# SiTronXD/vk3dGaussianSplatting

Hardware: AMD Instinct MI355X
Metric: Msplats/s + total frame ms (InitSortList/RadixSort/FindRanges/Render split) (higher is better)
Workload: dtype f32; 1 GPU; Garden-30k shape: 5,834,784 gaussians @ 1920x1080; num_gaussians=5834784, width=1920, height=1080, render_mode=exact, render_kernel=auto, sort_algorithm=radix4, frames_in_flight=1, parallelism=single GPU

## Files before the change

### vk3dgaussiansplatting_amd/csrc/gs_debug.cpp

```cpp
#include "gs_ctx.h"

using namespace gs;

extern "C" {

int gs_debug_init_sort_list(gs_ctx* c, const float view[16], const float proj[16],
                            const float cam_pos[3], uint32_t sh_mode) {
    if (!c) return GS_ERR_INVALID;
    const bool outputs_valid = c->outputs_valid;
    list_launching(c);
    if (!c->n || !c->capacity) return fail(c, GS_ERR_NO_SCENE, "gs_debug_init_sort_list: scene/resolution not set");
    if (!view || !proj || !cam_pos || sh_mode > 2u) return fail(c, GS_ERR_INVALID, "gs_debug_init_sort_list: bad argument");
    HIP_TRY(c, hipSetDevice(c->device));
    FrameParams fp = make_frame_params(c, view, proj, cam_pos, sh_mode);
    fp.parity = (c->emit_parity ^= 1u);
    launch_project(fp, c->scene, c->scratch, c->stream);
    launch_scan_blocks(fp, c->scratch, c->sort.params, c->ranges, c->sort.coarse, c->stream);
    launch_emit(fp, c->scratch, c->sort, c->stream);
    if (int r = check_launch(c, "InitSortList")) return r;
    HIP_TRY(c, hipStreamSynchronize(c->stream));
    unsorted_list_ready(c, fp, outputs_valid);
    SortParams sp{};
    HIP_TRY(c, hipMemcpy(&sp, c->sort.params, sizeof(sp), hipMemcpyDeviceToHost));
    return sp.overflow ? GS_WARN_OVERFLOW : GS_OK;
}

static int read_tile_words(gs_ctx* c, const uint32_t* dev, uint32_t num_elems, void* dst, size_t bytes) {
    if (bytes > (size_t)num_elems * sizeof(uint32_t)) return fail(c, GS_ERR_INVALID, "gs_debug_read: size exceeds buffer");
    const size_t cnt = bytes / sizeof(uint32_t);
    uint32_t* out = static_cast<uint32_t*>(dst);
    if (c->hi16) {
        std::vector<uint16_t> h(num_elems);
        if (num_elems) HIP_TRY(c, hipMemcpy(h.data(), dev, (size_t)num_elems * sizeof(uint16_t), hipMemcpyDeviceToHost));
        for (size_t i = 0; i < cnt; ++i) out[i] = h[i];
    } else if (cnt) {
        HIP_TRY(c, hipMemcpy(out, dev, cnt * sizeof(uint32_t), hipMemcpyDeviceToHost));
    }
    for (size_t i = 0; i < cnt; ++i) {
        const uint32_t k = out[i] / c->grid_w, x = out[i] - k * c->grid_w;
        out[i] = (c->first_row + k * c->row_stride) * c->grid_w + x;
    }
    return GS_OK;
}

int gs_debug_read(gs_ctx* c, int which, void* dst, size_t bytes) {
    if (!c || !dst) return GS_ERR_INVALID;
    HIP_TRY(c, hipSetDevice(c->device));
    HIP_TRY(c, hipStreamSynchronize(c->stream));
    if (c->last.kind == LastFrame::kNone && which != GS_BUF_IMAGE) return fail(c, GS_ERR_NO_SCENE, "gs_debug_read: no frame rendered yet");
    SortParams sp{};
    HIP_TRY(c, hipMemcpy(&sp, c->sort.params, sizeof(sp), hipMemcpyDeviceToHost));
    const size_t e_bytes = (size_t)sp.num_elems * sizeof(uint32_t);
    const void* src = nullptr;
    size_t avail = 0;
    const int si = c->last.sorted_index;
    switch (which) {
        case GS_BUF_SORTED_TILE:
            return read_tile_words(c, c->sort.hi[si], sp.num_elems, dst, bytes);
        case GS_BUF_SORTED_DEPTH:
            if (c->last.kind == LastFrame::kFrame && c->cfg.sort_algorithm != GS_SORT_TILE_BUCKET) {
                if (bytes > e_bytes) return fail(c, GS_ERR_INVALID, "gs_debug_read: size exceeds buffer");
                std::vector<uint32_t> ids(sp.num_elems), depth(c->n);
                if (sp.num_elems) HIP_TRY(c, hipMemcpy(ids.data(), c->sort.id[si], e_bytes, hipMemcpyDeviceToHost));
                HIP_TRY(c, hipMemcpy(depth.data(), c->scratch.depth_key, (size_t)c->n * sizeof(uint32_t), hipMemcpyDeviceToHost));
                uint32_t* out = static_cast<uint32_t*>(dst);
                for (size_t i = 0; i < bytes / sizeof(uint32_t); ++i) out[i] = ids[i] < c->n ? depth[ids[i]] : 0u;
                return GS_OK;
            }
            src = c->sort.lo[si]; avail = e_bytes; break;
        case GS_BUF_SORTED_ID: src = c->sort.id[si]; avail = e_bytes; break;
        case GS_BUF_RANGES: src = c->ranges; avail = (size_t)c->grid_w * c->grid_h * 8; break;
        case GS_BUF_COUNT: {
            if (bytes > sizeof(uint64_t)) return fail(c, GS_ERR_INVALID, "gs_debug_read: size");
            std::memcpy(dst, &sp.counter, bytes);
            return GS_OK;
        }
        case GS_BUF_IMAGE: src = c->framebuffer; avail = (size_t)c->width * c->height * 4; break;
        case GS_BUF_UNSORTED_TILE:
        case GS_BUF_UNSORTED_DEPTH:
        case GS_BUF_UNSORTED_ID:
            if (c->last.kind != LastFrame::kUnsortedList)
                return fail(c, GS_ERR_INVALID, "gs_debug_read: unsorted list only valid after gs_debug_init_sort_list");
            if (which == GS_BUF_UNSORTED_TILE) return read_tile_words(c, c->sort.hi[0], sp.num_elems, dst, bytes);
            src = which == GS_BUF_UNSORTED_DEPTH ? c->sort.lo[0] : c->sort.id[0];
            avail = e_bytes;
            break;
        case GS_BUF_COLOR:
        case GS_BUF_COV: {
            const size_t need = (size_t)c->n * 4 * sizeof(float);
            if (bytes > need) return fail(c, GS_ERR_INVALID, "gs_debug_read: size exceeds buffer");
            std::vector<SplatRaster> host(c->n);
            HIP_TRY(c, hipMemcpy(host.data(), c->scratch.raster, (size_t)c->n * sizeof(SplatRaster), hipMemcpyDeviceToHost));
            std::vector<float> opacity;
            std::vector<uint32_t> touched;
            std::vector<float> on_demand;
            const bool whole_grid = c->row_begin == 0u && c->row_end == c->grid_h && c->row_stride == 1u;
            if (which == GS_BUF_COLOR) {
                opacity.resize(c->n); touched.resize(c->n);
                HIP_TRY(c, hipMemcpy(opacity.data(), c->scene.opacity, (size_t)c->n * sizeof(float), hipMemcpyDeviceToHost));
                HIP_TRY(c, hipMemcpy(touched.data(), c->scratch.tiles_touched, (size_t)c->n * sizeof(uint32_t), hipMemcpyDeviceToHost));
                if (whole_grid) {
                    float* dev = nullptr;
                    HIP_TRY(c, hipMalloc((void**)&dev, need));
                    launch_debug_colour(c->last.fp, c->scene, c->scratch, dev, c->stream);
                    hipError_t e = hipGetLastError();
                    if (e == hipSuccess) e = hipStreamSynchronize(c->stream);
                    on_demand.resize((size_t)c->n * 4);
                    if (e == hipSuccess) e = hipMemcpy(on_demand.data(), dev, need, hipMemcpyDeviceToHost);
                    (void)hipFree(dev);
                    HIP_TRY(c, e);
                }
            }
            std::vector<uint8_t> wrote((size_t)c->num_blocks * 4);
            HIP_TRY(c, hipMemcpy(wrote.data(), c->scratch.wave_wrote, wrote.size(), hipMemcpyDeviceToHost));
            std::vector<float> outv((size_t)c->n * 4, 0.0f);
            for (uint32_t i = 0; i < c->n; ++i) {
                if (!wrote[i / 64u]) continue;
                const SplatRaster& r = host[i];
                float* o = &outv[(size_t)i * 4];
                if (which == GS_BUF_COLOR) {
                    if (touched[i]) { o[0] = r.r; o[1] = r.g; o[2] = r.b; o[3] = opacity[i]; }
                    else if (!on_demand.empty() && on_demand[(size_t)i * 4 + 3] != 0.0f) {
                        o[0] = on_demand[(size_t)i * 4]; o[1] = on_demand[(size_t)i * 4 + 1]; o[2] = on_demand[(size_t)i * 4 + 2]; o[3] = opacity[i];
                    }
                }
                else { o[0] = r.cx; o[1] = r.cy; o[2] = r.cz; o[3] = 0.0f; }
            }
            std::memcpy(dst, outv.data(), bytes);
            return GS_OK;
        }
        default: return fail(c, GS_ERR_INVALID, "gs_debug_read: unknown buffer id");
    }
    if (bytes > avail) return fail(c, GS_ERR_INVALID, "gs_debug_read: size exceeds buffer");
    if (bytes) HIP_TRY(c, hipMemcpy(dst, src, bytes, hipMemcpyDeviceToHost));
    return GS_OK;
}

int gs_sort_host(gs_ctx* c, uint32_t* tile, uint32_t* depth, uint32_t* id, uint32_t n,
                 uint32_t num_sort_bits) {
    if (!c || !tile || !depth || !id) return GS_ERR_INVALID;
    if (num_sort_bits == 0 || num_sort_bits > 64 || (num_sort_bits % kRadixBits) != 0)
        return fail(c, GS_ERR_INVALID, "gs_sort_host: num_sort_bits must be a multiple of 4 in [4,64]");
    if (n == 0) return GS_OK;
    HIP_TRY(c, hipSetDevice(c->device));
    SortBuffers sb{};
    DeviceOwner mem;
    int rc = alloc_sort(c, mem, sb, n);
    if (rc != GS_OK) { mem.release(); return rc; }
    const size_t bytes = (size_t)n * sizeof(uint32_t);
    hipError_t e = hipMemcpyAsync(sb.hi[0], tile, bytes, hipMemcpyHostToDevice, c->stream);
    if (e == hipSuccess) e = hipMemcpyAsync(sb.lo[0], depth, bytes, hipMemcpyHostToDevice, c->stream);
    if (e == hipSuccess) e = hipMemcpyAsync(sb.id[0], id, bytes, hipMemcpyHostToDevice, c->stream);
    int si = 0;
    if (e == hipSuccess) {
        launch_set_sort_params(sb.params, sb.coarse, n, c->stream);
        si = launch_radix_sort(sb, whole_list_run(c, n, num_sort_bits), c->stream);
        e = si < 0 ? hipErrorInvalidValue : hipGetLastError();
    }
    if (e == hipSuccess) e = hipMemcpyAsync(tile, sb.hi[si], bytes, hipMemcpyDeviceToHost, c->stream);
    if (e == hipSuccess) e = hipMemcpyAsync(depth, sb.lo[si], bytes, hipMemcpyDeviceToHost, c->stream);
    if (e == hipSuccess) e = hipMemcpyAsync(id, sb.id[si], bytes, hipMemcpyDeviceToHost, c->stream);
    if (e == hipSuccess) e = hipStreamSynchronize(c->stream);
    mem.release();
    if (e != hipSuccess) return fail(c, GS_ERR_HIP, std::string("gs_sort_host: ") + hipGetErrorString(e));
    return GS_OK;
}

int gs_sort_bench(gs_ctx* c, uint32_t n, uint32_t num_tiles, uint32_t iters, uint64_t seed,
                  float* ms_per_sort, uint32_t* sorted_ok) {
    if (!c || !ms_per_sort || n == 0 || num_tiles == 0 || iters == 0) return GS_ERR_INVALID;
    HIP_TRY(c, hipSetDevice(c->device));
    SortBuffers sb{};
    DeviceOwner mem;
    int rc = alloc_sort(c, mem, sb, n);
    if (rc != GS_OK) { mem.release(); return rc; }
    const SortRun run = whole_list_run(c, n, num_sort_bits_for(num_tiles));
    uint32_t* bad = nullptr;
    hipEvent_t e0 = nullptr, e1 = nullptr;
    hipError_t e = mem.alloc(bad, sizeof(uint32_t));
    if (e == hipSuccess) e = hipEventCreate(&e0);
    if (e == hipSuccess) e = hipEventCreate(&e1);
    float total_ms = 0.0f;
    int si = 0;
    for (uint32_t it = 0; it < iters + 1 && e == hipSuccess; ++it) {
        launch_fill_random_keys(sb.lo[0], sb.hi[0], sb.id[0], n, num_tiles, seed + it, c->stream);
        launch_set_sort_params(sb.params, sb.coarse, n, c->stream);
        e = hipEventRecord(e0, c->stream);
        if (e != hipSuccess) break;
        si = launch_radix_sort(sb, run, c->stream);
        if (si < 0) { si = 0; e = hipErrorInvalidValue; break; }
        e = hipEventRecord(e1, c->stream);
        if (e == hipSuccess) e = hipStreamSynchronize(c->stream);
        float ms = 0.0f;
        if (e == hipSuccess) e = hipEventElapsedTime(&ms, e0, e1);
        if (it > 0) total_ms += ms;
    }
    uint32_t bad_host = 0;
    if (e == hipSuccess) e = hipMemsetAsync(bad, 0, sizeof(uint32_t), c->stream);
    if (e == hipSuccess) {
        launch_check_sorted(sb.lo[si], sb.hi[si], n, bad, c->stream);
        e = hipMemcpyAsync(&bad_host, bad, sizeof(uint32_t), hipMemcpyDeviceToHost, c->stream);
    }
    if (e == hipSuccess) e = hipStreamSynchronize(c->stream);
    if (e0) (void)hipEventDestroy(e0);
    if (e1) (void)hipEventDestroy(e1);
    mem.release();
    if (e != hipSuccess) return fail(c, GS_ERR_HIP, std::string("gs_sort_bench: ") + hipGetErrorString(e));
    *ms_per_sort = total_ms / (float)iters;
    if (sorted_ok) *sorted_ok = bad_host == 0 ? 1u : 0u;
// ... 39 lines not shown
```

### vk3dgaussiansplatting_amd/csrc/gs_internal.h

```cpp
#pragma once

#include <hip/hip_runtime.h>
#include <stdint.h>
#include "gs_record.h"

namespace gs {

constexpr int kWave = 64;
constexpr int kTile = 16;
constexpr int kRadixBits = 4;
constexpr int kBins = 1 << kRadixBits;

constexpr int kSortThreads = 256;
constexpr int kSortKeysPerThread = 8;
constexpr int kSortTile = kSortThreads * kSortKeysPerThread;
constexpr int kSegments = 512;
constexpr int kCoarse = 64;
constexpr int kMaxSortPasses = 16;
#ifndef GS_FED_MAX_GROUPS
#define GS_FED_MAX_GROUPS 1024
#endif
constexpr uint32_t kFedMaxGroups = GS_FED_MAX_GROUPS;

constexpr int kBins8 = 256;
// ... 67 lines not shown
    uint32_t* block_sums;
    uint32_t* block_offsets;
    uint2* help_list;
    uint32_t* help_count;
    uint32_t* help_slot;
    uint32_t* band_list;
    uint32_t* block_flags;
    uint32_t* flag_offsets;
    uint32_t* sorted_sums;
    SortParams* aux_params;
    uint32_t* elems_note;
    float* view_z;
};
#ifndef GS_EMIT_SLICE
#define GS_EMIT_SLICE 4096
#endif
constexpr uint32_t kEmitSlice = GS_EMIT_SLICE;
constexpr uint32_t kEmitHelpCap = 65536;
constexpr uint32_t kEmitNoHelp = 0xFFFFFFFFu;
__host__ __device__ inline uint32_t emit_helpers(uint32_t capacity) {
    const uint32_t by_capacity = capacity / kEmitSlice + 1u;
    return by_capacity < kEmitHelpCap ? by_capacity : kEmitHelpCap;
}

struct SortBuffers {
    uint32_t *lo[2], *hi[2], *id[2];
    uint32_t* table;
    uint32_t* seg_sum;
    uint32_t* coarse;
    uint32_t* fed[3];
    SortParams* params;
    uint32_t digit_bits;
};

struct SortRun {
    uint32_t capacity = 0;
    uint32_t first_bit = 0;
    uint32_t num_sort_bits = 0;
    int start = 0;
    uint32_t coarse_pass = 0;
    const SortParams* params = nullptr;
    bool drop_depth_payload = false;
    bool hi16 = false;
    float share = 1.0f;
    bool fed = false;
    hipEvent_t* scatter_events = nullptr;
};

struct SortPass {
    uint32_t shift;
    uint32_t bits, mask;
    bool tile_word;
    bool word16;
    uint32_t word_shift;
    int lo_in, lo_out;
    bool last;
};
inline uint32_t sort_pass_count(const SortRun& r, uint32_t digit_bits) {
    return r.num_sort_bits > r.first_bit ? (r.num_sort_bits - r.first_bit + digit_bits - 1u) / digit_bits : 0u;
}
inline SortPass sort_pass(const SortRun& r, uint32_t digit_bits, uint32_t k) {
    SortPass p{};
    p.shift = r.first_bit + k * digit_bits;
    p.bits = r.num_sort_bits - p.shift < digit_bits ? r.num_sort_bits - p.shift : digit_bits;
    p.mask = (1u << p.bits) - 1u;
    p.tile_word = p.shift >= 32u;
    p.last = p.shift + digit_bits >= r.num_sort_bits;
    p.lo_in = 4; p.lo_out = 4;
    if (r.drop_depth_payload) {
        if (p.tile_word) { p.lo_in = 0; p.lo_out = 0; }
        else if (r.first_bit == 0u) {
            p.lo_in = p.shift >= 16u ? 2 : 4;
            p.lo_out = p.shift + digit_bits >= 32u ? 0 : (p.shift + digit_bits >= 16u ? 2 : 4);
        }
    }
    const bool lo16 = !p.tile_word && p.lo_in == 2;
    p.word16 = (p.tile_word && r.hi16) || lo16;
    p.word_shift = lo16 ? p.shift - 16u : p.shift & 31u;
    return p;
}

void launch_project(const FrameParams& fp, const SceneBuffers& scene, const SplatScratch& sc,
                    hipStream_t stream);
void launch_debug_colour(const FrameParams& fp, const SceneBuffers& scene, const SplatScratch& sc, float* out_rgba, hipStream_t stream);
void launch_scan_blocks(const FrameParams& fp, const SplatScratch& sc, SortParams* params,
                        uint32_t* ranges, uint32_t* coarse, hipStream_t stream);
void launch_emit(const FrameParams& fp, const SplatScratch& sc, const SortBuffers& sb,
                 hipStream_t stream);
void launch_splat_list(const FrameParams& fp, const SplatScratch& sc, const SortBuffers& sb, hipStream_t stream);
void launch_gather_sorted(const FrameParams& fp, const SplatScratch& sc, const SortBuffers& sb, int sorted, hipStream_t stream);
void launch_emit_sorted(const FrameParams& fp, const SplatScratch& sc, const SortBuffers& sb, int sorted, hipStream_t stream);
int launch_radix_sort(const SortBuffers& sb, const SortRun& run, hipStream_t stream);
int launch_radix_sort8(const SortBuffers& sb, const SortRun& run, hipStream_t stream);
int init_tile_sort();
void launch_tile_sort(const FrameParams& fp, const uint32_t* ranges, uint32_t* lo, uint32_t* id,
                      uint32_t* lo_alt, uint32_t* id_alt, hipStream_t stream, hipStream_t helper = nullptr,
                      hipEvent_t fork = nullptr, hipEvent_t join = nullptr);
void launch_find_ranges(const FrameParams& fp, const uint32_t* sorted_tile, const SortParams* params,
                        uint32_t* ranges, hipStream_t stream);
void launch_tile_order(const FrameParams& fp, const uint32_t* ranges, uint32_t* order, hipStream_t stream);
size_t tile_order_words(uint32_t grid_w, uint32_t grid_h);
struct RenderOutputs {
    float4* rgba32f;
    float* depth;
    const float* view_z;
};
void launch_render(const FrameParams& fp, const SplatRaster* raster, const uint32_t* sorted_id,
                   const uint32_t* ranges, const uint32_t* order, uint8_t* rgba, uint32_t render_mode,
                   uint32_t render_kernel, hipStream_t stream, const RenderOutputs& outs = RenderOutputs{});
struct SplatScan {
    uint32_t* offsets;
    uint32_t* block_sums;
    uint32_t* block_offsets;
    uint32_t* totals;
};
constexpr int kRowFloats = 10;
struct BackwardBuffers {
    float* rows;
    SplatScan scan;
    uint32_t* vis_ids;
};
inline const uint32_t* visible_count_of(const BackwardBuffers& bb) { return bb.scan.totals + 1; }
inline size_t backward_row_bytes(uint32_t capacity) { return (size_t)capacity * kRowFloats * sizeof(float); }
inline uint32_t backward_blocks(uint32_t n) { return (n + 255u) / 256u; }
struct BackwardFrame {
    FrameParams fp;
    SceneBuffers scene;
    SplatScratch sc;
    const uint32_t* sorted_id;
    const uint32_t* ranges;
    BackwardBuffers bb;
};
void launch_backward(const BackwardFrame& f, const float* grad_rgba, const float* grad_depth, float* grad_records,
                     hipStream_t stream);
void launch_backward_visible_scan(const BackwardFrame& f, uint32_t* ids_out, uint32_t max_rows, uint32_t* count_out,
                                  hipStream_t stream);
void launch_backward_visible_rows(const BackwardFrame& f, const float* grad_rgba, const float* grad_depth,
                                  uint32_t max_rows, float* grad_rows, hipStream_t stream);
size_t backward_camera_partial_bytes(uint32_t n);
void launch_backward_camera(const BackwardFrame& f, float* partials, float* grad_camera, hipStream_t stream);
struct LossBuffers {
    float* maps;
    float* tile_sums;
};
size_t loss_map_bytes(uint32_t width, uint32_t height);
size_t loss_tile_bytes(uint32_t width, uint32_t height);
void launch_photometric_loss(const LossBuffers& lb, const float* rgba, const float* target, float lambda, const float* bg,
                             uint32_t width, uint32_t height, float* loss_out, float* grad, hipStream_t stream);
void launch_aos_to_soa(const float* chunk, uint32_t first, uint32_t count, uint32_t n,
                       const SceneBuffers& s, hipStream_t stream);
void launch_block_bounds(uint32_t n, const SceneBuffers& s, hipStream_t stream);
void launch_upload_rows(const float* records, uint32_t n, const uint32_t* ids, const uint32_t* count, uint32_t max_rows,
                        const SceneBuffers& s, hipStream_t stream);
struct AdamStep {
    float beta1, beta2, c1, c2, eps;
    float step[6], lo[6], hi[6];
};
void launch_adam_rows(float* records, float* m, float* v, uint32_t n, const uint32_t* ids, const float* grad_rows,
                      const uint32_t* count, uint32_t max_rows, const AdamStep& a, hipStream_t stream);
void launch_adam_rows_raw(float* raw, float* records, float* m, float* v, uint32_t n, const uint32_t* ids,
                          const float* grad_rows, const uint32_t* count, uint32_t max_rows, const AdamStep& a,
                          hipStream_t stream);
void launch_convert_space(const float* src, float* dst, uint32_t n, bool to_raw, hipStream_t stream);
void launch_reset_opacity_raw(float* raw, float* records, float* m, float* v, uint32_t n, float max_opacity, float logit,
                              hipStream_t stream);
struct DensifyStatsArgs {
    const uint32_t* ids;
// ... 55 lines not shown
```

### vk3dgaussiansplatting_amd/csrc/gs_project.hip

```cpp
#include <cstdlib>
#include "gs_splat_math.h"

namespace gs {

__device__ __forceinline__ Mat3 mat3_mul(const Mat3& a, const Mat3& b) {
    Mat3 c;
#pragma unroll
    for (int j = 0; j < 3; ++j)
#pragma unroll
        for (int i = 0; i < 3; ++i) {
            float acc = a.m[0][i] * b.m[j][0];
            acc = acc + a.m[1][i] * b.m[j][1];
            acc = acc + a.m[2][i] * b.m[j][2];
            c.m[j][i] = acc;
        }
    return c;
}
__device__ __forceinline__ Mat3 mat3_transpose(const Mat3& a) {
    Mat3 t;
#pragma unroll
    for (int j = 0; j < 3; ++j)
#pragma unroll
        for (int i = 0; i < 3; ++i) t.m[j][i] = a.m[i][j];
    return t;
// ... 176 lines not shown
    const bool survives = leader && mask != 0xFu;
    if (leader && !survives) {
        sc.block_sums[b] = 0u;
        if (fp.splat_first) sc.block_flags[b] = 0u;
        reinterpret_cast<uint32_t*>(sc.wave_wrote)[b] = 0u;
    }
    const uint64_t vote = __ballot(survives);
    if (lane == 0) s_cnt[wave] = (uint32_t)__builtin_popcountll(vote);
    __syncthreads();
    uint32_t before = 0u, total = 0u;
#pragma unroll
    for (int w = 0; w < kCullThreads / 64; ++w) {
        const uint32_t c = s_cnt[w];
        before += w < wave ? c : 0u;
        total += c;
    }
    if (total == 0u) return;
    if (threadIdx.x == 0) s_base = atomicAdd(&sc.help_count[2u + fp.parity], total);
    __syncthreads();
    if (survives)
        sc.band_list[s_base + before + (uint32_t)__builtin_popcountll(vote & ((1ull << lane) - 1ull))] = b | (mask << 28);
}

template <bool NT>
__device__ __forceinline__ float sh_load(const float* p) { return NT ? __builtin_nontemporal_load(p) : *p; }

template <bool NT>
__device__ __forceinline__ void splat_colour(const FrameParams& fp, const float* shp, const uint32_t n, const float px, const float py,
                                             const float pz, float res[3]) {
    const float ddx = px - fp.cam_pos[0], ddy = py - fp.cam_pos[1], ddz = pz - fp.cam_pos[2];
    const float len = sqrtf(ddx * ddx + ddy * ddy + ddz * ddz);
    float basis[16];
    sh_eval4(ddx / len, ddy / len, ddz / len, basis);
    res[0] = 0.0f; res[1] = 0.0f; res[2] = 0.0f;
    if (fp.sh_mode == 0u) {
#pragma unroll
        for (int i = 0; i < 16; ++i)
#pragma unroll
            for (int c = 0; c < 3; ++c)
                res[c] = res[c] + sh_load<NT>(shp + (size_t)(i * 3 + c) * n) * basis[i];
    } else if (fp.sh_mode == 1u) {
#pragma unroll
        for (int i = 1; i < 16; ++i)
#pragma unroll
            for (int c = 0; c < 3; ++c)
                res[c] = res[c] + sh_load<NT>(shp + (size_t)(i * 3 + c) * n) * basis[i];
#pragma unroll
        for (int c = 0; c < 3; ++c) res[c] = res[c] - 0.5f;
    } else if (fp.sh_mode == 2u) {
#pragma unroll
        for (int c = 0; c < 3; ++c) res[c] = res[c] + sh_load<NT>(shp + (size_t)c * n) * basis[0];
    }
#pragma unroll
    for (int c = 0; c < 3; ++c) {
        res[c] = res[c] + 0.5f;
        res[c] = maxf(res[c], 0.0f);
    }
}

#ifndef GS_PROJECT_MINBLOCKS
#define GS_PROJECT_MINBLOCKS 7
#endif
template <bool NT_SH, bool VIEW_Z>
__global__ __launch_bounds__(kProjThreads, GS_PROJECT_MINBLOCKS) void k_project(const FrameParams fp,
                                                           const SceneBuffers scene,
                                                           const SplatScratch sc, const uint32_t num_blocks) {
    __shared__ uint32_t s_wave_sum[kProjThreads / 64];
    __shared__ uint32_t s_wave_emits[kProjThreads / 64];
    __shared__ uint32_t s_wave_flags[kProjThreads / 64];
    __shared__ float4 s_raster[kProjThreads * 3];
    const uint32_t n = fp.num_gaussians;
    const bool band = !owns_every_row(fp);
    const bool listed = band && fp.row_stride == 1u;
    uint32_t blk = blockIdx.x;
    bool wave_skip = false;
    if (listed) {
        if (blk >= sc.help_count[2u + fp.parity]) return;
        const uint32_t rec = sc.band_list[blk];
        blk = rec & 0x0FFFFFFFu;
        wave_skip = ((rec >> 28) >> wave_id()) & 1u;
    }
    const uint32_t g = blk * kProjThreads + threadIdx.x;
    uint32_t count = 0;
    bool kept = false;
    float4 rec0 = make_float4(0.f, 0.f, 0.f, 0.f), rec1 = rec0, rec2 = rec0;

    if (g < n && !wave_skip) {
        const float px = scene.pos[g], py = scene.pos[(size_t)n + g], pz = scene.pos[2 * (size_t)n + g];
        float vp[4];
        mat4_mul_vec4(fp.view, px, py, pz, 1.0f, vp);
        if (!(-vp[2] <= fp.near_plane)) {
            float q[4];
            mat4_mul_vec4(fp.proj, vp[0], vp[1], vp[2], vp[3], q);
            const float ndc_x = q[0] / q[3];
            const float ndc_y = q[1] / q[3];
            if (!(fabsf(ndc_x) > fp.ndc_cull || fabsf(ndc_y) > fp.ndc_cull)) {
                float nd = (-vp[2] - fp.near_plane) / (fp.far_plane - fp.near_plane);
                nd = clampf(nd, 0.0f, 1.0f);
                const uint32_t depth_key = f2u_sat(nd * 4294967296.0f);
                bool band_skip = false;

                if (band) {
                    const float hgt = (float)fp.height;
                    const float tfx = fp.tan_fov_y * (float)fp.width / hgt;
                    const float tx = clampf(vp[0] / vp[2], -tfx * fp.in_view_limit, tfx * fp.in_view_limit);
                    const float ty = clampf(vp[1] / vp[2], -fp.tan_fov_y * fp.in_view_limit, fp.tan_fov_y * fp.in_view_limit);
                    const float rmax = radius_bound(fp, tx, ty, vp[2], scene.sig2[g]);
                    const float sy_b = (1.0f - ndc_y) * 0.5f * hgt;
                    band_skip = misses_owned_rows(fp, sy_b - rmax, sy_b + rmax);
                }
                if (!band_skip) {
                    float scale[3], rot[4], cov[3];
#pragma unroll
                    for (int a = 0; a < 3; ++a) scale[a] = scene.scale[a * (size_t)n + g];
#pragma unroll
                    for (int a = 0; a < 4; ++a) rot[a] = scene.rot[a * (size_t)n + g];
                    get_covariance(fp, scale, rot, vp, cov);

                    float sx = ndc_x, sy = -ndc_y;
                    sx = (sx + 1.0f) * 0.5f;
                    sy = (sy + 1.0f) * 0.5f;
                    sx = sx * (float)fp.width;
                    sy = sy * (float)fp.height;

                    const float det = cov[0] * cov[2] - cov[1] * cov[1];
                    const float radius = tile_extent_radius(cov[0], cov[1], cov[2]);
                    const int gw = (int)fp.grid_w, gh = (int)fp.grid_h;
                    const int min_x = clampi(f2i_sat((sx - radius) / 16.0f), 0, gw);
                    const int min_y = clampi(f2i_sat((sy - radius) / 16.0f), 0, gh);
                    int tx = f2i_sat((sx + radius) / 16.0f);
                    int ty = f2i_sat((sy + radius) / 16.0f);
                    const int max_x = clampi(tx == 2147483647 ? tx : tx + 1, 0, gw);
                    const int max_y = clampi(ty == 2147483647 ? ty : ty + 1, 0, gh);

                    int y0 = min_y > (int)fp.row_begin ? min_y : (int)fp.row_begin;
                    int y1 = max_y < (int)fp.row_end ? max_y : (int)fp.row_end;
                    if (y1 < y0) y1 = y0;
                    const int k0 = owned_rows_below(fp, y0), k1 = owned_rows_below(fp, y1);
                    count = (uint32_t)(max_x - min_x) * (uint32_t)(k1 - k0);

                    kept = true;
                    rec0 = make_float4(sx, sy, 0.0f, 0.0f);
                    rec2 = make_float4(0.0f, cov[0], cov[1], cov[2]);
                    if (count != 0u) {
                        float opacity = scene.opacity[g];
                        float inv_x = 0.0f, inv_y = 0.0f, inv_z = 0.0f;
                        if (det != 0.0f) {
                            const float det_inv = 1.0f / det;
                            inv_x = cov[2] * det_inv;
                            inv_y = -cov[1] * det_inv;
                            inv_z = cov[0] * det_inv;
                        } else {
                            opacity = 0.0f;
                        }
                        rec0.z = inv_x; rec0.w = inv_y;
                        rec2.x = opacity;
                        float res[3];
                        splat_colour<NT_SH>(fp, scene.sh + g, n, px, py, pz, res);
                        rec1 = make_float4(inv_z, res[0], res[1], res[2]);
                        sc.depth_key[g] = depth_key;
                        if constexpr (VIEW_Z) sc.view_z[g] = -vp[2];
                        sc.extents[g] = make_uint2((uint32_t)min_x | ((uint32_t)k0 << 16),
                                                   (uint32_t)max_x | ((uint32_t)k1 << 16));
                    }
                }
            }
        }
        sc.tiles_touched[g] = count;
    } else if (g < n) {
        sc.tiles_touched[g] = 0u;
    }

    s_raster[threadIdx.x * 3 + 0] = rec0;
    s_raster[threadIdx.x * 3 + 1] = rec1;
    s_raster[threadIdx.x * 3 + 2] = rec2;
    const uint32_t wsum = wave_sum_to_lane63(count);
    const uint32_t wflags = (uint32_t)__popcll(__ballot(count != 0u));
    const bool wave_kept = __ballot(kept) != 0ull;
    if (lane_id() == 63) {
        s_wave_sum[wave_id()] = wsum;
        s_wave_flags[wave_id()] = wflags;
#ifndef GS_PROJECT_WRITE_ALL
#define GS_PROJECT_WRITE_ALL 0
#endif
        const uint32_t wrote = (band ? wsum != 0u : (GS_PROJECT_WRITE_ALL || wave_kept)) ? 1u : 0u;
        s_wave_emits[wave_id()] = wrote;
        sc.wave_wrote[blk * (kProjThreads / 64) + wave_id()] = (uint8_t)wrote;
    }
    __syncthreads();
    {
        const uint32_t first = blk * kProjThreads;
        const uint32_t valid = (n - first) < (uint32_t)kProjThreads ? (n - first) : (uint32_t)kProjThreads;
        float4* out = reinterpret_cast<float4*>(sc.raster + first);
#pragma unroll
        for (int q = 0; q < 3; ++q) {
            const uint32_t i = q * kProjThreads + threadIdx.x;
            if (i < valid * 3u && s_wave_emits[i / 192u]) out[i] = s_raster[i];
        }
    }
    uint32_t t = 0;
#pragma unroll
    for (int w = 0; w < kProjThreads / 64; ++w) t += s_wave_sum[w];
    if (threadIdx.x == 0) {
        sc.block_sums[blk] = t;
        if (fp.splat_first) sc.block_flags[blk] = s_wave_flags[0] + s_wave_flags[1] + s_wave_flags[2] + s_wave_flags[3];
    }
    if (!fp.splat_first) register_emit_helpers(fp, sc, blk, t);
}

struct ScanJob { const uint32_t* sums; uint32_t* offsets; SortParams* params; uint32_t capacity;
                 uint32_t* host_note; };
constexpr uint32_t kScanClearWgs = 8;
__global__ __launch_bounds__(1024) void k_scan_blocks(const ScanJob job0, const ScanJob job1, uint32_t jobs, uint32_t num_blocks,
                                                       uint4* __restrict__ zero_a, uint32_t n16_a,
                                                       uint4* __restrict__ zero_b, uint32_t n16_b,
                                                       uint32_t* __restrict__ next_help_count) {
    if (blockIdx.x >= jobs) {
        const uint32_t k = blockIdx.x - jobs;
        if (k == 0u && threadIdx.x == 0 && next_help_count) { next_help_count[0] = 0u; next_help_count[2] = 0u; }
        for (uint32_t i = k * 1024u + threadIdx.x; i < n16_a; i += kScanClearWgs * 1024u) zero_a[i] = make_uint4(0u, 0u, 0u, 0u);
        for (uint32_t i = k * 1024u + threadIdx.x; i < n16_b; i += kScanClearWgs * 1024u) zero_b[i] = make_uint4(0u, 0u, 0u, 0u);
        return;
    }
    const ScanJob job = blockIdx.x == 0 ? job0 : job1;
    const uint32_t* __restrict__ block_sums = job.sums;
    uint32_t* __restrict__ block_offsets = job.offsets;
    SortParams* params = job.params;
    const uint32_t capacity = job.capacity;
    __shared__ uint64_t s_wave_tot[16];
    const int tid = threadIdx.x, lane = tid & 63, wave = tid >> 6;
    const uint32_t per = (((num_blocks + 1023u) / 1024u) + 3u) & ~3u;
    const uint4* in4 = reinterpret_cast<const uint4*>(block_sums + (size_t)tid * per);
    uint4* out4 = reinterpret_cast<uint4*>(block_offsets + (size_t)tid * per);
    auto sat = [](uint64_t x) { return (uint32_t)(x > 0xFFFFFFFFull ? 0xFFFFFFFFull : x); };
    constexpr uint32_t kHeld = 8;
    const bool held = per / 4 <= kHeld;
    uint4 v[kHeld];
    uint64_t sum = 0;
    if (held) {
#pragma unroll
        for (uint32_t i = 0; i < kHeld; ++i) v[i] = i < per / 4 ? in4[i] : make_uint4(0u, 0u, 0u, 0u);
#pragma unroll
        for (uint32_t i = 0; i < kHeld; ++i) sum += (uint64_t)v[i].x + v[i].y + v[i].z + v[i].w;
    } else {
#pragma unroll 4
        for (uint32_t i = 0; i < per / 4; ++i) {
            const uint4 w = in4[i];
            sum += (uint64_t)w.x + w.y + w.z + w.w;
        }
    }
    const uint64_t inc = wave_inclusive_scan64(sum);
    if (lane == 63) s_wave_tot[wave] = inc;
    __syncthreads();
    uint64_t run = inc - sum;
    for (int w = 0; w < wave; ++w) run += s_wave_tot[w];
    if (tid == 1023) {
        const uint64_t counter = run + sum;
        const uint32_t e = counter < capacity ? (uint32_t)counter : capacity;
        params->counter = counter;
        params->num_elems = e;
        params->num_groups = (e + kSortTile - 1) / kSortTile;
        params->groups_per_seg = (params->num_groups + kSegments - 1) / kSegments;
        params->overflow = counter > capacity ? 1u : 0u;
        if (job.host_note) __hip_atomic_store(job.host_note, e + 1u, __ATOMIC_RELAXED, __HIP_MEMORY_SCOPE_SYSTEM);
    }
    if (held) {
#pragma unroll
        for (uint32_t i = 0; i < kHeld; ++i) {
// ... 80 lines not shown
    __syncthreads();

    const uint32_t g0 = blk * kProjThreads;
    const uint32_t my_excl = s_incl[tid] - cnt;
    const uint32_t c_begin = slice * kEmitSlice;
    const uint32_t c_end = alone || total - c_begin < kEmitSlice ? total : c_begin + kEmitSlice;
    for (uint32_t c0 = c_begin; c0 < c_end; c0 += kEmitChunk) {
#pragma unroll
        for (int k = 0; k < kEmitChunk / kProjThreads; ++k) s_owner[k * kProjThreads + tid] = 0u;
        __syncthreads();
        if (cnt != 0u) {
            if (my_excl >= c0) {
                if (my_excl - c0 < (uint32_t)kEmitChunk) s_owner[my_excl - c0] = (uint32_t)tid + 1u;
            } else if (my_excl + cnt > c0) {
                s_owner[0] = (uint32_t)tid + 1u;
            }
        }
        __syncthreads();
        uint4 o = *reinterpret_cast<const uint4*>(&s_owner[4 * tid]);
        o.y = o.y > o.x ? o.y : o.x;
        o.z = o.z > o.y ? o.z : o.y;
        o.w = o.w > o.z ? o.w : o.z;
        const uint32_t winc = wave_inclusive_max(o.w);
        if (lane_id() == 63) s_wmax[wave_id()] = winc;
        uint32_t prev = __shfl_up(winc, 1, 64);
        if (lane_id() == 0) prev = 0u;
        __syncthreads();
        for (int w = 0; w < wave_id(); ++w) prev = prev > s_wmax[w] ? prev : s_wmax[w];
        o.x = o.x > prev ? o.x : prev;
        o.y = o.y > prev ? o.y : prev;
        o.z = o.z > prev ? o.z : prev;
        o.w = o.w > prev ? o.w : prev;
        *reinterpret_cast<uint4*>(&s_owner[4 * tid]) = o;
        __syncthreads();
#pragma unroll
        for (int k = 0; k < kEmitChunk / kProjThreads; ++k) {
            const uint32_t jj = (uint32_t)(k * kProjThreads + tid);
            const uint32_t j = c0 + jj;
            if (j < total) {
                const uint32_t s = s_owner[jj] - 1u;
                const uint32_t excl = s > 0u ? s_incl[s - 1u] : 0u;
                const uint32_t id_local = j - excl;
                const uint2 ext = s_ext[s];
                const uint32_t min_x = ext.x & 0xFFFFu, y0 = ext.x >> 16, max_x = ext.y & 0xFFFFu;
                const uint32_t wdt = max_x - min_x;
                uint32_t ry = (uint32_t)((float)id_local * __builtin_amdgcn_rcpf((float)wdt));
                int32_t rx = (int32_t)(id_local - ry * wdt);
                if (rx < 0) { --ry; rx += (int32_t)wdt; }
                else if ((uint32_t)rx >= wdt) { ++ry; rx -= (int32_t)wdt; }
                const uint32_t tile_key = (y0 + ry) * fp.grid_w + (min_x + (uint32_t)rx);
                const uint64_t out = (uint64_t)base + j;
                if (out < fp.capacity) {
                    if (fp.hi16) reinterpret_cast<uint16_t*>(out_hi)[out] = (uint16_t)tile_key;
                    else out_hi[out] = tile_key;
                    if constexpr (SORTED) out_id[out] = s_depth[s];
                    else { out_lo[out] = s_depth[s]; out_id[out] = g0 + s; }
                }
            }
        }
        __syncthreads();
    }
}

void launch_project(const FrameParams& fp, const SceneBuffers& scene, const SplatScratch& sc,
                    hipStream_t stream) {
    const uint32_t blocks = (fp.num_gaussians + kProjThreads - 1) / kProjThreads;
    if (blocks == 0) return;
    const bool listed = !(fp.row_begin == 0u && fp.row_end == fp.grid_h) && fp.row_stride == 1u;
    if (listed) hipLaunchKernelGGL(k_band_cull, dim3((blocks * 4u + (uint32_t)kCullThreads - 1u) / (uint32_t)kCullThreads), dim3(kCullThreads), 0, stream,
                                   fp, scene, sc, blocks);
#ifndef GS_PROJECT_NT_SH_ABOVE
#define GS_PROJECT_NT_SH_ABOVE ((size_t)256u << 20)
#endif
    const bool nt_sh = (size_t)fp.num_gaussians * 236u > GS_PROJECT_NT_SH_ABOVE;
    if (sc.view_z) {
        if (nt_sh) hipLaunchKernelGGL((k_project<true, true>), dim3(blocks), dim3(kProjThreads), 0, stream, fp, scene, sc, blocks);
        else hipLaunchKernelGGL((k_project<false, true>), dim3(blocks), dim3(kProjThreads), 0, stream, fp, scene, sc, blocks);
    } else {
        if (nt_sh) hipLaunchKernelGGL((k_project<true, false>), dim3(blocks), dim3(kProjThreads), 0, stream, fp, scene, sc, blocks);
        else hipLaunchKernelGGL((k_project<false, false>), dim3(blocks), dim3(kProjThreads), 0, stream, fp, scene, sc, blocks);
    }
}

__global__ __launch_bounds__(256) void k_debug_colour(const FrameParams fp, const SceneBuffers scene, const SplatScratch sc, float4* out) {
    const uint32_t n = fp.num_gaussians;
    const uint32_t g = blockIdx.x * 256u + threadIdx.x;
    if (g >= n) return;
    float4 o = make_float4(0.f, 0.f, 0.f, 0.f);
    if (sc.wave_wrote[g >> 6] && sc.raster[g].cx != 0.0f && sc.tiles_touched[g] == 0u) {
        float res[3];
        splat_colour<false>(fp, scene.sh + g, n, scene.pos[g], scene.pos[(size_t)n + g], scene.pos[2 * (size_t)n + g], res);
        o = make_float4(res[0], res[1], res[2], 1.0f);
    }
    out[g] = o;
}

void launch_debug_colour(const FrameParams& fp, const SceneBuffers& scene, const SplatScratch& sc, float* out_rgba, hipStream_t stream) {
    const uint32_t blocks = (fp.num_gaussians + 255u) / 256u;
    if (blocks) hipLaunchKernelGGL(k_debug_colour, dim3(blocks), dim3(256), 0, stream, fp, scene, sc, reinterpret_cast<float4*>(out_rgba));
}

void launch_scan_blocks(const FrameParams& fp, const SplatScratch& sc, SortParams* params,
                        uint32_t* ranges, uint32_t* coarse, hipStream_t stream) {
    const uint32_t blocks = (fp.num_gaussians + kProjThreads - 1) / kProjThreads;
    const uint32_t n16_ranges = (fp.grid_w * fp.grid_h * 2u + 3u) / 4u;
    const uint32_t n16_coarse = (uint32_t)(kMaxSortPasses * kBins * kCoarse) / 4u;
    const ScanJob elements{sc.block_sums, sc.block_offsets, params, fp.capacity, sc.elems_note};
    const ScanJob splats{sc.block_flags, sc.flag_offsets, sc.aux_params, fp.num_gaussians, nullptr};
    const uint32_t jobs = fp.splat_first ? 2u : 1u;
    hipLaunchKernelGGL(k_scan_blocks, dim3(jobs + kScanClearWgs), dim3(1024), 0, stream, elements, splats, jobs, blocks,
                       reinterpret_cast<uint4*>(ranges), n16_ranges, reinterpret_cast<uint4*>(coarse), n16_coarse,
                       sc.help_count + (fp.parity ^ 1u));
}

void launch_emit(const FrameParams& fp, const SplatScratch& sc, const SortBuffers& sb,
                 hipStream_t stream) {
    const uint32_t blocks = (fp.num_gaussians + kProjThreads - 1) / kProjThreads;
    if (blocks == 0) return;
    const uint32_t helpers = emit_helpers(fp.capacity);
    hipLaunchKernelGGL((k_emit<false>), dim3(helpers + blocks), dim3(kProjThreads), 0, stream, fp, sc, sb.lo[0],
                       sb.hi[0], sb.id[0], blocks, helpers, (const uint32_t*)nullptr, (const uint32_t*)nullptr);
}

__global__ __launch_bounds__(kProjThreads) void k_splat_list(const FrameParams fp, const SplatScratch sc,
                                                              uint32_t* __restrict__ out_depth, uint32_t* __restrict__ out_count,
                                                              uint32_t* __restrict__ out_id) {
    __shared__ uint32_t s_cnt[kProjThreads / 64], s_flag[kProjThreads / 64];
    const uint32_t blk = blockIdx.x, g = blk * kProjThreads + threadIdx.x;
    if (blk == 0u && threadIdx.x == 0u) sc.help_count[fp.parity] = 0u;
    if (sc.block_sums[blk] == 0u) return;
    const uint32_t cnt = g < fp.num_gaussians ? sc.tiles_touched[g] : 0u;
    const uint32_t dk = cnt != 0u ? sc.depth_key[g] : 0u;
    const uint64_t off0 = sc.block_offsets[blk];
    const uint32_t fpos0 = sc.flag_offsets[blk];
    const uint32_t inc = wave_inclusive_scan(cnt);
    const uint64_t fb = __ballot(cnt != 0u);
    if (lane_id() == 63) { s_cnt[wave_id()] = inc; s_flag[wave_id()] = (uint32_t)__popcll(fb); }
    __syncthreads();
    uint64_t off = off0 + (inc - cnt);
    uint32_t pos = fpos0 + (uint32_t)__popcll(fb & ((1ull << lane_id()) - 1ull));
    for (int w = 0; w < wave_id(); ++w) { off += s_cnt[w]; pos += s_flag[w]; }
    if (cnt != 0u) {
        const uint64_t room = off < fp.capacity ? (uint64_t)fp.capacity - off : 0ull;
        const uint32_t kept = room < cnt ? (uint32_t)room : cnt;
        out_depth[pos] = dk;
        if (fp.hi16) reinterpret_cast<uint16_t*>(out_count)[pos] = (uint16_t)kept;
        else out_count[pos] = kept;
        out_id[pos] = g;
    }
}

constexpr int kSumsBlocksPerWg = 8;
__global__ __launch_bounds__(kProjThreads) void k_sorted_sums(const FrameParams fp, const SplatScratch sc,
                                                               const uint32_t* __restrict__ sorted_counts, uint32_t num_blocks) {
    const uint32_t ve = sc.aux_params[0].num_elems;
    const int lane = lane_id();
#pragma unroll
    for (int it = 0; it < kSumsBlocksPerWg / (kProjThreads / 64); ++it) {
        const uint32_t blk = blockIdx.x * kSumsBlocksPerWg + (uint32_t)(it * (kProjThreads / 64) + wave_id());
        if (blk >= num_blocks) return;
        const uint32_t i0 = blk * kProjThreads + 4u * (uint32_t)lane;
        uint32_t c[4] = {0u, 0u, 0u, 0u};
        if (i0 + 3u < ve) {
            if (fp.hi16) {
                const uint2 v = *reinterpret_cast<const uint2*>(reinterpret_cast<const uint16_t*>(sorted_counts) + i0);
                c[0] = v.x & 0xFFFFu; c[1] = v.x >> 16; c[2] = v.y & 0xFFFFu; c[3] = v.y >> 16;
            } else {
                const uint4 v = *reinterpret_cast<const uint4*>(sorted_counts + i0);
                c[0] = v.x; c[1] = v.y; c[2] = v.z; c[3] = v.w;
            }
        } else {
#pragma unroll
            for (int k = 0; k < 4; ++k)
                if (i0 + k < ve) c[k] = fp.hi16 ? (uint32_t)reinterpret_cast<const uint16_t*>(sorted_counts)[i0 + k] : sorted_counts[i0 + k];
        }
        const uint32_t t = (uint32_t)__builtin_amdgcn_readlane((int)wave_sum_to_lane63(c[0] + c[1] + c[2] + c[3]), 63);
        if (lane == 0) sc.sorted_sums[blk] = t;
        if (t > kEmitSlice) {
            const uint32_t extra = (t - 1u) / kEmitSlice;
            uint32_t slot = 0u;
            if (lane == 0) {
                slot = atomicAdd(&sc.help_count[fp.parity], extra);
// ... 36 lines not shown
```

Before: 5985 Msplats/s.

## Write projected splat records only for waves that emit tiles, recompute debug records lazily

```diff
diff --git a/vk3dgaussiansplatting_amd/csrc/gs_debug.cpp b/vk3dgaussiansplatting_amd/csrc/gs_debug.cpp
--- a/vk3dgaussiansplatting_amd/csrc/gs_debug.cpp
+++ b/vk3dgaussiansplatting_amd/csrc/gs_debug.cpp
@@ -92,39 +92,45 @@
             std::vector<SplatRaster> host(c->n);
             HIP_TRY(c, hipMemcpy(host.data(), c->scratch.raster, (size_t)c->n * sizeof(SplatRaster), hipMemcpyDeviceToHost));
             std::vector<float> opacity;
-            std::vector<uint32_t> touched;
-            std::vector<float> on_demand;
-            const bool whole_grid = c->row_begin == 0u && c->row_end == c->grid_h && c->row_stride == 1u;
             if (which == GS_BUF_COLOR) {
-                opacity.resize(c->n); touched.resize(c->n);
+                opacity.resize(c->n);
                 HIP_TRY(c, hipMemcpy(opacity.data(), c->scene.opacity, (size_t)c->n * sizeof(float), hipMemcpyDeviceToHost));
-                HIP_TRY(c, hipMemcpy(touched.data(), c->scratch.tiles_touched, (size_t)c->n * sizeof(uint32_t), hipMemcpyDeviceToHost));
-                if (whole_grid) {
-                    float* dev = nullptr;
-                    HIP_TRY(c, hipMalloc((void**)&dev, need));
-                    launch_debug_colour(c->last.fp, c->scene, c->scratch, dev, c->stream);
-                    hipError_t e = hipGetLastError();
-                    if (e == hipSuccess) e = hipStreamSynchronize(c->stream);
-                    on_demand.resize((size_t)c->n * 4);
-                    if (e == hipSuccess) e = hipMemcpy(on_demand.data(), dev, need, hipMemcpyDeviceToHost);
-                    (void)hipFree(dev);
-                    HIP_TRY(c, e);
+            }
+            std::vector<uint32_t> touched(c->n);
+            HIP_TRY(c, hipMemcpy(touched.data(), c->scratch.tiles_touched, (size_t)c->n * sizeof(uint32_t), hipMemcpyDeviceToHost));
+            std::vector<float> cov_od((size_t)c->n * 4), col_od;
+            {
+                const bool colour = which == GS_BUF_COLOR;
+                float* dev = nullptr;
+                HIP_TRY(c, hipMalloc((void**)&dev, need * (colour ? 2 : 1)));
+                float* dev_col = colour ? dev + (size_t)c->n * 4 : nullptr;
+                launch_debug_records(c->last.fp, c->scene, c->scratch, dev, dev_col, c->stream);
+                hipError_t e = hipGetLastError();
+                if (e == hipSuccess) e = hipStreamSynchronize(c->stream);
+                if (e == hipSuccess) e = hipMemcpy(cov_od.data(), dev, need, hipMemcpyDeviceToHost);
+                if (colour) {
+                    col_od.resize((size_t)c->n * 4);
+                    if (e == hipSuccess) e = hipMemcpy(col_od.data(), dev_col, need, hipMemcpyDeviceToHost);
                 }
+                (void)hipFree(dev);
+                HIP_TRY(c, e);
             }
             std::vector<uint8_t> wrote((size_t)c->num_blocks * 4);
             HIP_TRY(c, hipMemcpy(wrote.data(), c->scratch.wave_wrote, wrote.size(), hipMemcpyDeviceToHost));
             std::vector<float> outv((size_t)c->n * 4, 0.0f);
             for (uint32_t i = 0; i < c->n; ++i) {
-                if (!wrote[i / 64u]) continue;
                 const SplatRaster& r = host[i];
                 float* o = &outv[(size_t)i * 4];
+                const bool emitted = wrote[i / 64u] && touched[i];
+                const float* od = &cov_od[(size_t)i * 4];
+                if (!emitted && od[3] == 0.0f) continue;
                 if (which == GS_BUF_COLOR) {
-                    if (touched[i]) { o[0] = r.r; o[1] = r.g; o[2] = r.b; o[3] = opacity[i]; }
-                    else if (!on_demand.empty() && on_demand[(size_t)i * 4 + 3] != 0.0f) {
-                        o[0] = on_demand[(size_t)i * 4]; o[1] = on_demand[(size_t)i * 4 + 1]; o[2] = on_demand[(size_t)i * 4 + 2]; o[3] = opacity[i];
-                    }
+                    if (emitted) { o[0] = r.r; o[1] = r.g; o[2] = r.b; }
+                    else { o[0] = col_od[(size_t)i * 4]; o[1] = col_od[(size_t)i * 4 + 1]; o[2] = col_od[(size_t)i * 4 + 2]; }
+                    o[3] = opacity[i];
                 }
-                else { o[0] = r.cx; o[1] = r.cy; o[2] = r.cz; o[3] = 0.0f; }
+                else if (emitted) { o[0] = r.cx; o[1] = r.cy; o[2] = r.cz; }
+                else { o[0] = od[0]; o[1] = od[1]; o[2] = od[2]; }
             }
             std::memcpy(dst, outv.data(), bytes);
             return GS_OK;
diff --git a/vk3dgaussiansplatting_amd/csrc/gs_internal.h b/vk3dgaussiansplatting_amd/csrc/gs_internal.h
--- a/vk3dgaussiansplatting_amd/csrc/gs_internal.h
+++ b/vk3dgaussiansplatting_amd/csrc/gs_internal.h
@@ -173,7 +173,8 @@
 
 void launch_project(const FrameParams& fp, const SceneBuffers& scene, const SplatScratch& sc,
                     hipStream_t stream);
-void launch_debug_colour(const FrameParams& fp, const SceneBuffers& scene, const SplatScratch& sc, float* out_rgba, hipStream_t stream);
+void launch_debug_records(const FrameParams& fp, const SceneBuffers& scene, const SplatScratch& sc, float* out_cov, float* out_rgba,
+                          hipStream_t stream);
 void launch_scan_blocks(const FrameParams& fp, const SplatScratch& sc, SortParams* params,
                         uint32_t* ranges, uint32_t* coarse, hipStream_t stream);
 void launch_emit(const FrameParams& fp, const SplatScratch& sc, const SortBuffers& sb,
diff --git a/vk3dgaussiansplatting_amd/csrc/gs_project.hip b/vk3dgaussiansplatting_amd/csrc/gs_project.hip
--- a/vk3dgaussiansplatting_amd/csrc/gs_project.hip
+++ b/vk3dgaussiansplatting_amd/csrc/gs_project.hip
@@ -282,7 +282,6 @@
     }
     const uint32_t g = blk * kProjThreads + threadIdx.x;
     uint32_t count = 0;
-    bool kept = false;
     float4 rec0 = make_float4(0.f, 0.f, 0.f, 0.f), rec1 = rec0, rec2 = rec0;
 
     if (g < n && !wave_skip) {
@@ -339,7 +338,6 @@
                     const int k0 = owned_rows_below(fp, y0), k1 = owned_rows_below(fp, y1);
                     count = (uint32_t)(max_x - min_x) * (uint32_t)(k1 - k0);
 
-                    kept = true;
                     rec0 = make_float4(sx, sy, 0.0f, 0.0f);
                     rec2 = make_float4(0.0f, cov[0], cov[1], cov[2]);
                     if (count != 0u) {
@@ -376,14 +374,13 @@
     s_raster[threadIdx.x * 3 + 2] = rec2;
     const uint32_t wsum = wave_sum_to_lane63(count);
     const uint32_t wflags = (uint32_t)__popcll(__ballot(count != 0u));
-    const bool wave_kept = __ballot(kept) != 0ull;
     if (lane_id() == 63) {
         s_wave_sum[wave_id()] = wsum;
         s_wave_flags[wave_id()] = wflags;
 #ifndef GS_PROJECT_WRITE_ALL
 #define GS_PROJECT_WRITE_ALL 0
 #endif
-        const uint32_t wrote = (band ? wsum != 0u : (GS_PROJECT_WRITE_ALL || wave_kept)) ? 1u : 0u;
+        const uint32_t wrote = ((GS_PROJECT_WRITE_ALL && !band) || wsum != 0u) ? 1u : 0u;
         s_wave_emits[wave_id()] = wrote;
         sc.wave_wrote[blk * (kProjThreads / 64) + wave_id()] = (uint8_t)wrote;
     }
@@ -630,22 +627,47 @@
     }
 }
 
-__global__ __launch_bounds__(256) void k_debug_colour(const FrameParams fp, const SceneBuffers scene, const SplatScratch sc, float4* out) {
+__global__ __launch_bounds__(256) void k_debug_records(const FrameParams fp, const SceneBuffers scene, const SplatScratch sc,
+                                                       float4* out_cov, float4* out_col) {
     const uint32_t n = fp.num_gaussians;
     const uint32_t g = blockIdx.x * 256u + threadIdx.x;
     if (g >= n) return;
-    float4 o = make_float4(0.f, 0.f, 0.f, 0.f);
-    if (sc.wave_wrote[g >> 6] && sc.raster[g].cx != 0.0f && sc.tiles_touched[g] == 0u) {
-        float res[3];
-        splat_colour<false>(fp, scene.sh + g, n, scene.pos[g], scene.pos[(size_t)n + g], scene.pos[2 * (size_t)n + g], res);
-        o = make_float4(res[0], res[1], res[2], 1.0f);
-    }
-    out[g] = o;
-}
-
-void launch_debug_colour(const FrameParams& fp, const SceneBuffers& scene, const SplatScratch& sc, float* out_rgba, hipStream_t stream) {
+    float4 ocov = make_float4(0.f, 0.f, 0.f, 0.f), ocol = ocov;
+    const bool emits = sc.wave_wrote[g >> 6] && sc.tiles_touched[g] != 0u;
+    if (!emits) {
+        const float px = scene.pos[g], py = scene.pos[(size_t)n + g], pz = scene.pos[2 * (size_t)n + g];
+        float vp[4];
+        mat4_mul_vec4(fp.view, px, py, pz, 1.0f, vp);
+        if (!(-vp[2] <= fp.near_plane)) {
+            float q[4];
+            mat4_mul_vec4(fp.proj, vp[0], vp[1], vp[2], vp[3], q);
+            const float ndc_x = q[0] / q[3];
+            const float ndc_y = q[1] / q[3];
+            if (!(fabsf(ndc_x) > fp.ndc_cull || fabsf(ndc_y) > fp.ndc_cull)) {
+                float scale[3], rot[4], cov[3];
+#pragma unroll
+                for (int a = 0; a < 3; ++a) scale[a] = scene.scale[a * (size_t)n + g];
+#pragma unroll
+                for (int a = 0; a < 4; ++a) rot[a] = scene.rot[a * (size_t)n + g];
+                get_covariance(fp, scale, rot, vp, cov);
+                ocov = make_float4(cov[0], cov[1], cov[2], 1.0f);
+                if (out_col) {
+                    float res[3];
+                    splat_colour<false>(fp, scene.sh + g, n, px, py, pz, res);
+                    ocol = make_float4(res[0], res[1], res[2], 1.0f);
+                }
+            }
+        }
+    }
+    out_cov[g] = ocov;
+    if (out_col) out_col[g] = ocol;
+}
+
+void launch_debug_records(const FrameParams& fp, const SceneBuffers& scene, const SplatScratch& sc, float* out_cov, float* out_rgba,
+                          hipStream_t stream) {
     const uint32_t blocks = (fp.num_gaussians + 255u) / 256u;
-    if (blocks) hipLaunchKernelGGL(k_debug_colour, dim3(blocks), dim3(256), 0, stream, fp, scene, sc, reinterpret_cast<float4*>(out_rgba));
+    if (blocks) hipLaunchKernelGGL(k_debug_records, dim3(blocks), dim3(256), 0, stream, fp, scene, sc, reinterpret_cast<float4*>(out_cov),
+                                   reinterpret_cast<float4*>(out_rgba));
 }
 
 void launch_scan_blocks(const FrameParams& fp, const SplatScratch& sc, SortParams* params,
```

Measured after the change: 6049 Msplats/s, median of 6. +1.1%, better.
